# YurongYou/MODEST

Measured on AMD Instinct MI355X. Metric: LiDAR scans/sec through PP-score+cluster seed-label pipeline, higher is better.
Workload: dtype f64

## Files before the change

modest_amd/csrc/cluster.hip:

```cpp
#include "common.h"
#include "compact.h"
#include "mask_pred.h"
#include <cmath>

using namespace modest;

namespace {

constexpr int CG = 128;
constexpr int CG_CELLS = CG * CG;
constexpr int WPB = 4;
constexpr int KNN_KEYS = 1024;
constexpr double D_INF = __builtin_huge_val();

struct CGrid {
    double ox, oy, inv_c;
};

__device__ __forceinline__ int cg_coord(float v, double o, double inv_c) {
    double f = floor(((double)v - o) * inv_c);
    f = fmin(fmax(f, 0.0), (double)(CG - 1));
    return (int)f;
}

__global__ __launch_bounds__(1024) void cg_bbox(const float *__restrict__ xyz, int n, double c, CGrid *g,
                                                unsigned *__restrict__ zeroed, int zero_words) {
    for (int i = threadIdx.x; i < zero_words; i += blockDim.x) zeroed[i] = 0u;
    float mnx = INFINITY, mny = INFINITY, mxx = -INFINITY, mxy = -INFINITY;
    for (int i = threadIdx.x; i < n; i += blockDim.x) {
        const float x = xyz[3 * (size_t)i], y = xyz[3 * (size_t)i + 1];
        mnx = fminf(mnx, x);
        mxx = fmaxf(mxx, x);
        mny = fminf(mny, y);
        mxy = fmaxf(mxy, y);
    }
    for (int o = 32; o > 0; o >>= 1) {
        mnx = fminf(mnx, __shfl_xor(mnx, o));
        mxx = fmaxf(mxx, __shfl_xor(mxx, o));
        mny = fminf(mny, __shfl_xor(mny, o));
        mxy = fmaxf(mxy, __shfl_xor(mxy, o));
    }
    __shared__ float s[4][16];
    const int w = threadIdx.x >> 6, l = threadIdx.x & 63;
    if (l == 0) {
        s[0][w] = mnx;
        s[1][w] = mxx;
        s[2][w] = mny;
        s[3][w] = mxy;
    }
    __syncthreads();
    if (threadIdx.x == 0) {
        for (int k = 1; k < 16; ++k) {
            s[0][0] = fminf(s[0][0], s[0][k]);
            s[1][0] = fmaxf(s[1][0], s[1][k]);
            s[2][0] = fminf(s[2][0], s[2][k]);
            s[3][0] = fmaxf(s[3][0], s[3][k]);
        }
        double cx = 0.5 * ((double)s[0][0] + (double)s[1][0]);
        double cy = 0.5 * ((double)s[2][0] + (double)s[3][0]);
        if (!(cx == cx) || fabs(cx) > 1e30) cx = 0.0;
        if (!(cy == cy) || fabs(cy) > 1e30) cy = 0.0;
        g->ox = cx - 0.5 * CG * c;
        g->oy = cy - 0.5 * CG * c;
        g->inv_c = 1.0 / c;
    }
}

__global__ void cg_count(const float *__restrict__ xyz, int n, const CGrid *g, unsigned *cnt) {
    const int i = blockIdx.x * blockDim.x + threadIdx.x;
    if (i >= n) return;
    const int cx = cg_coord(xyz[3 * (size_t)i], g->ox, g->inv_c);
    const int cy = cg_coord(xyz[3 * (size_t)i + 1], g->oy, g->inv_c);
    atomicAdd(&cnt[cy * CG + cx], 1u);
}

constexpr int SCAN_IPT = 8;
template <bool CELLS>
__device__ __forceinline__ void scan_u32_body(const unsigned *in, unsigned *__restrict__ out, int n,
                                              unsigned *__restrict__ total_copy, const int *__restrict__ flag_src,
                                              unsigned *__restrict__ cursor, unsigned *clear_in, unsigned *flags) {
    __shared__ unsigned tile[16][64 * (SCAN_IPT + 1)];
    __shared__ unsigned wtot[2][16];
    const int lane = threadIdx.x & 63, w = threadIdx.x >> 6;
    unsigned *T = tile[w];
    unsigned carry = 0;
    int buf = 0;
    for (int t0 = 0; t0 < n; t0 += 1024 * SCAN_IPT, buf ^= 1) {
        const int seg = t0 + w * 64 * SCAN_IPT;
        unsigned v[SCAN_IPT];
#pragma unroll
        for (int q = 0; q < SCAN_IPT; ++q) {
            const int e = q * 64 + lane;
            v[q] = seg + e < n ? in[seg + e] : 0u;
        }
#pragma unroll
// ... 49 lines not shown
        out[n] = carry;
        if (total_copy) {
            total_copy[0] = flag_src ? (unsigned)*flag_src : 0u;
            total_copy[1] = carry;
        }
    }
}
template <bool CELLS>
__global__ __launch_bounds__(1024) void scan_u32(const unsigned *in, unsigned *__restrict__ out, int n,
                                                 unsigned *__restrict__ total_copy = nullptr,
                                                 const int *__restrict__ flag_src = nullptr,
                                                 unsigned *__restrict__ cursor = nullptr,
                                                 unsigned *clear_in = nullptr, unsigned *flags = nullptr) {
    scan_u32_body<CELLS>(in, out, n, total_copy, flag_src, cursor, clear_in, flags);
}

__device__ __forceinline__ void cg_scatter_body(const float *__restrict__ xyz, const float *__restrict__ pp, int n, const CGrid *g, unsigned *cursor, float4 *__restrict__ sorted, int *__restrict__ sidx, const int *__restrict__ idx, const float *__restrict__ inten_src, const float *__restrict__ rows, int stride, float *__restrict__ sortedI, const unsigned bx, const unsigned gx) {
    const int i = bx * blockDim.x + threadIdx.x;
    if (i >= n) return;
    const float x = xyz[3 * (size_t)i], y = xyz[3 * (size_t)i + 1], z = xyz[3 * (size_t)i + 2];
    const int cell = cg_coord(y, g->oy, g->inv_c) * CG + cg_coord(x, g->ox, g->inv_c);
    const unsigned slot = atomicAdd(&cursor[cell], 1u);
    const int src = idx ? idx[i] : i;
    sorted[slot] = make_float4(x, y, z, pp[src]);
    sidx[slot] = i;
    if (sortedI) sortedI[slot] = rows ? rows[(size_t)src * stride + 3] : inten_src[src];
}
__global__  void cg_scatter(const float *__restrict__ xyz, const float *__restrict__ pp, int n, const CGrid *g, unsigned *cursor, float4 *__restrict__ sorted, int *__restrict__ sidx, const int *__restrict__ idx, const float *__restrict__ inten_src, const float *__restrict__ rows, int stride, float *__restrict__ sortedI) {
    cg_scatter_body(xyz, pp, n, g, cursor, sorted, sidx, idx, inten_src, rows, stride, sortedI, blockIdx.x, gridDim.x);
}

__device__ __forceinline__ void mask_count_kernel_body(const float *__restrict__ pts, int n, int stride, MaskParams P, CGrid G, CGrid *__restrict__ g, unsigned *cnt, int *__restrict__ labels, float *__restrict__ kept, int *__restrict__ kept_idx, unsigned long long *state, int *n_kept, const unsigned bx, const unsigned gx) {
    const unsigned blk = compact_ticket(state);
    const long long i = (long long)blk * 1024 + threadIdx.x;
    if (blk == 0 && threadIdx.x == 0) *g = G;
    bool keep = false;
    float x = 0, y = 0, z = 0;
    if (i < n) {
        const float *p = pts + i * stride;
        x = p[0];
        y = p[1];
        z = p[2];
        keep = mask_keep(P, x, y, z);
        labels[i] = -1;
        if (keep) atomicAdd(&cnt[cg_coord(y, G.oy, G.inv_c) * CG + cg_coord(x, G.ox, G.inv_c)], 1u);
    }
    const unsigned long long dst = compact_offset(keep, blk, gx, state, n_kept);
    if (keep) {
        kept[3 * dst + 0] = x;
        kept[3 * dst + 1] = y;
        kept[3 * dst + 2] = z;
        kept_idx[dst] = (int)i;
    }
}
__global__ __launch_bounds__(1024) void mask_count_kernel(const float *__restrict__ pts, int n, int stride, MaskParams P, CGrid G, CGrid *__restrict__ g, unsigned *cnt, int *__restrict__ labels, float *__restrict__ kept, int *__restrict__ kept_idx, unsigned long long *state, int *n_kept) {
    mask_count_kernel_body(pts, n, stride, P, G, g, cnt, labels, kept, kept_idx, state, n_kept, blockIdx.x, gridDim.x);
}

__device__ __forceinline__ double dist2(const float4 &a, const float4 &b) {
    const double dx = (double)a.x - (double)b.x;
    const double dy = (double)a.y - (double)b.y;
    const double dz = (double)a.z - (double)b.z;
    return __dadd_rn(__dadd_rn(__dmul_rn(dx, dx), __dmul_rn(dy, dy)), __dmul_rn(dz, dz));
}

struct Rows {
    static constexpr int n = 3;
    unsigned s[3], e[3];
};
__device__ __forceinline__ Rows rows_of(const float4 &q, const CGrid *g, const unsigned *__restrict__ start) {
    const int cx = cg_coord(q.x, g->ox, g->inv_c), cy = cg_coord(q.y, g->oy, g->inv_c);
    const int x0 = max(cx - 1, 0), x1 = min(cx + 1, CG - 1);
    Rows r;
#pragma unroll
    for (int d = 0; d < 3; ++d) {
        const int yy = cy - 1 + d;
        const bool ok = yy >= 0 && yy < CG;
        r.s[d] = ok ? start[yy * CG + x0] : 0u;
        r.e[d] = ok ? start[yy * CG + x1 + 1] : 0u;
    }
    return r;
}

__device__ __forceinline__ void knn_kth_kernel_body(const float4 *__restrict__ sorted, int n, const CGrid *g, const unsigned *__restrict__ start, int k, double r2, double *__restrict__ kthS, const unsigned bx, const unsigned gx) {
    __shared__ unsigned hist_all[WPB][256];
    __shared__ unsigned keys_all[WPB][KNN_KEYS];
    const int w = threadIdx.x >> 6, lane = threadIdx.x & 63;
    const int s = bx * WPB + w;
    if (s >= n) return;
    unsigned *hist = hist_all[w];
    unsigned *keys = keys_all[w];
    const float4 q = sorted[s];
    const Rows R = rows_of(q, g, start);
    unsigned prefix = 0, mask = 0, cntF = 0;
    int kk = k - 1;
    bool enough = true;
    unsigned nkeys = 0;
    for (int shift = 24; shift >= 0; shift -= 8) {
        for (int b = lane; b < 256; b += 64) hist[b] = 0;
        __builtin_amdgcn_wave_barrier();
        if (shift == 24) {
    #pragma unroll
    for (int r = 0; r < R.n; ++r)
            for (unsigned base = R.s[r]; base < R.e[r]; base += 64) {
                const unsigned j = base + lane;
                bool inr = false;
                unsigned key = 0;
                if (j < R.e[r] && (int)j != s) {
                    const double d2 = dist2(q, sorted[j]);
                    inr = d2 <= r2;
                    key = __float_as_uint((float)d2);
                }
                const unsigned long long bal = __ballot(inr);
                if (inr) {
                    atomicAdd(&hist[(key >> 24) & 255u], 1u);
                    const unsigned pos = nkeys + (unsigned)__popcll(bal & ((1ULL << lane) - 1ULL));
                    if (pos < (unsigned)KNN_KEYS) keys[pos] = key;
                }
                nkeys += (unsigned)__popcll(bal);
            }
        } else if (nkeys <= (unsigned)KNN_KEYS) {
            for (unsigned i = lane; i < nkeys; i += 64) {
                const unsigned key = keys[i];
                if ((key & mask) == prefix) atomicAdd(&hist[(key >> shift) & 255u], 1u);
            }
        } else {
    #pragma unroll
    for (int r = 0; r < R.n; ++r)
            for (unsigned j = R.s[r] + lane; j < R.e[r]; j += 64) {
                if ((int)j == s) continue;
                const double d2 = dist2(q, sorted[j]);
                if (d2 <= r2) {
                    const unsigned key = __float_as_uint((float)d2);
                    if ((key & mask) == prefix) atomicAdd(&hist[(key >> shift) & 255u], 1u);
                }
            }
        }
        __builtin_amdgcn_wave_barrier();
        const unsigned c0 = hist[4 * lane], c1 = hist[4 * lane + 1], c2 = hist[4 * lane + 2],
                       c3 = hist[4 * lane + 3];
        const unsigned mine = c0 + c1 + c2 + c3;
        unsigned inc = mine;
        for (int o = 1; o < 64; o <<= 1) {
            const unsigned v = __shfl_up(inc, o);
            if (lane >= o) inc += v;
        }
        const unsigned total = __shfl(inc, 63);
        if (shift == 24 && total < (unsigned)k) {
            enough = false;
            break;
        }
        const unsigned long long bal = __ballot(inc > (unsigned)kk);
        const int owner = __ffsll((long long)bal) - 1;
        const unsigned excl = __shfl(inc - mine, owner);
        const unsigned o0 = __shfl(c0, owner), o1 = __shfl(c1, owner), o2 = __shfl(c2, owner),
                       o3 = __shfl(c3, owner);
        int rem = kk - (int)excl;
        int bin = 4 * owner;
        cntF = o0;
        if (rem >= (int)o0) {
            rem -= o0;
            ++bin;
            cntF = o1;
            if (rem >= (int)o1) {
                rem -= o1;
                ++bin;
                cntF = o2;
                if (rem >= (int)o2) {
                    rem -= o2;
                    ++bin;
                    cntF = o3;
                }
            }
        }
        kk = rem;
        prefix |= (unsigned)bin << shift;
        mask |= 255u << shift;
        __builtin_amdgcn_wave_barrier();
    }
    double result = D_INF;
    if (enough) {
        double lo = -1.0;
        for (;;) {
            double m = D_INF;
        #pragma unroll
    for (int r = 0; r < R.n; ++r)
                for (unsigned j = R.s[r] + lane; j < R.e[r]; j += 64) {
                    if ((int)j == s) continue;
                    const double d2 = dist2(q, sorted[j]);
                    if (d2 <= r2 && d2 > lo && __float_as_uint((float)d2) == prefix) m = fmin(m, d2);
                }
            for (int o = 32; o > 0; o >>= 1) m = fmin(m, __shfl_xor(m, o));
            if (cntF == 1) {
                result = m;
                break;
            }
            unsigned c = 0;
        #pragma unroll
    for (int r = 0; r < R.n; ++r)
                for (unsigned j = R.s[r] + lane; j < R.e[r]; j += 64)
                    if ((int)j != s && dist2(q, sorted[j]) == m) ++c;
            for (int o = 32; o > 0; o >>= 1) c += __shfl_xor(c, o);
            if (kk < (int)c || c == 0) {
                result = m;
                break;
            }
            kk -= (int)c;
            lo = m;
        }
    }
    if (lane == 0) kthS[s] = result;
}
__global__ __launch_bounds__(64 * WPB) void knn_kth_kernel(const float4 *__restrict__ sorted, int n, const CGrid *g, const unsigned *__restrict__ start, int k, double r2, double *__restrict__ kthS) {
    knn_kth_kernel_body(sorted, n, g, start, k, r2, kthS, blockIdx.x, gridDim.x);
}

struct EdgeP {
    double r2, eps;
    int use_knn, affinity;
    const float *inten;
};

__device__ __forceinline__ bool weight_ok(const float4 &q, const float4 &c, const EdgeP &ep, int s, unsigned j) {
    float w;
    if (ep.affinity == 0) {
        w = fabsf(q.w - c.w);
    } else if (ep.affinity == 1) {
        const float d = q.w - c.w;
        w = (float)exp((double)(d * d));
    } else {
        const float dx = q.x - c.x, dy = q.y - c.y, dz = q.z - c.z, di = ep.inten[s] - ep.inten[j];
        w = sqrtf(((dx * dx + dy * dy) + dz * dz) + di * di);
    }
    return (double)w <= ep.eps;
}

__device__ __forceinline__ bool edge_ok(const float4 &q, double kq, const float4 &c, double kc, const EdgeP &ep,
                                        int s, unsigned j) {
    const double d2 = dist2(q, c);
    const double lim = ep.use_knn ? fmin(fmin(kq, kc), ep.r2) : ep.r2;
    if (!(d2 <= lim)) return false;
    return weight_ok(q, c, ep, s, j);
}

__global__ __launch_bounds__(64 * WPB) void degree_kernel(const float4 *__restrict__ sorted, int n,
                                                          const CGrid *g,
                                                          const unsigned *__restrict__ start,
                                                          const double *__restrict__ kthS, EdgeP ep, int min_samples,
                                                          unsigned char *__restrict__ coreS) {
    const int w = threadIdx.x >> 6, lane = threadIdx.x & 63;
    const int s = blockIdx.x * WPB + w;
    if (s >= n) return;
    const float4 q = sorted[s];
    const double kq = kthS[s];
    const Rows R = rows_of(q, g, start);
    unsigned cnt = 0;
#pragma unroll
    for (int r = 0; r < R.n; ++r)
        for (unsigned j = R.s[r] + lane; j < R.e[r]; j += 64) {
            if ((int)j == s) continue;
            if (edge_ok(q, kq, sorted[j], kthS[j], ep, s, j)) ++cnt;
        }
    for (int o = 32; o > 0; o >>= 1) cnt += __shfl_xor(cnt, o);
    if (lane == 0) coreS[s] = ((int)cnt + 1 >= min_samples) ? 1 : 0;
}

__device__ __forceinline__ int uf_load(int *p, int i) {
    return __hip_atomic_load(p + i, __ATOMIC_RELAXED, __HIP_MEMORY_SCOPE_AGENT);
}
__device__ __forceinline__ int uf_find(int *parent, int x) {
    int p = uf_load(parent, x);
    while (p != x) {
        const int gp = uf_load(parent, p);
        if (gp != p) __hip_atomic_store(parent + x, gp, __ATOMIC_RELAXED, __HIP_MEMORY_SCOPE_AGENT);
        x = p;
        p = gp;
    }
    return x;
}
__device__ __forceinline__ void uf_unite(int *parent, int a, int b) {
    for (;;) {
        a = uf_find(parent, a);
        b = uf_find(parent, b);
        if (a == b) return;
        if (a > b) {
            const int t = a;
            a = b;
            b = t;
        }
        const int old = atomicCAS(parent + b, b, a);
        if (old == b) return;
    }
}

__global__ void uf_init(int *parent, int n) {
    const int i = blockIdx.x * blockDim.x + threadIdx.x;
    if (i < n) parent[i] = i;
}

__global__ __launch_bounds__(64 * WPB) void hook_min_kernel(const float4 *__restrict__ sorted, int n,
                                                            const CGrid *g,
                                                            const unsigned *__restrict__ start,
                                                            const double *__restrict__ kthS,
                                                            const unsigned char *__restrict__ coreS,
                                                            const int *__restrict__ sidx, EdgeP ep, int *parent) {
    const int w = threadIdx.x >> 6, lane = threadIdx.x & 63;
    const int s = blockIdx.x * WPB + w;
    if (s >= n) return;
    if (!coreS[s]) return;
    const float4 q = sorted[s];
    const double kq = kthS[s];
    const int me = sidx[s];
    const Rows R = rows_of(q, g, start);
    int best = me;
#pragma unroll
    for (int r = 0; r < R.n; ++r)
        for (unsigned j = R.s[r] + lane; j < R.e[r]; j += 64) {
            if ((int)j == s || !coreS[j]) continue;
            const int other = sidx[j];
            if (other < best && edge_ok(q, kq, sorted[j], kthS[j], ep, s, j)) best = other;
        }
    for (int o = 32; o > 0; o >>= 1) best = min(best, __shfl_xor(best, o));
    if (lane == 0) parent[me] = best;
}

__global__ __launch_bounds__(64 * WPB) void union_kernel(const float4 *__restrict__ sorted, int n,
                                                         const CGrid *g,
                                                         const unsigned *__restrict__ start,
                                                         const double *__restrict__ kthS,
                                                         const unsigned char *__restrict__ coreS,
                                                         const int *__restrict__ sidx, EdgeP ep, int *parent) {
    const int w = threadIdx.x >> 6, lane = threadIdx.x & 63;
    const int s = blockIdx.x * WPB + w;
    if (s >= n) return;
    if (!coreS[s]) return;
    const float4 q = sorted[s];
    const double kq = kthS[s];
    const int me = sidx[s];
    const Rows R = rows_of(q, g, start);
#pragma unroll
    for (int r = 0; r < R.n; ++r)
        for (unsigned j = R.s[r] + lane; j < R.e[r]; j += 64) {
            if ((int)j <= s) continue;
            if (!coreS[j]) continue;
            if (edge_ok(q, kq, sorted[j], kthS[j], ep, s, j)) uf_unite(parent, me, sidx[j]);
        }
}

__global__ void compress_kernel(int *parent, const unsigned char *__restrict__ coreS,
                                const int *__restrict__ sidx, int n, int *__restrict__ root,
                                unsigned *__restrict__ isroot) {
    const int s = blockIdx.x * blockDim.x + threadIdx.x;
    if (s >= n) return;
    const int i = sidx[s];
    const int r = uf_find(parent, i);
    root[i] = r;
    isroot[i] = (coreS[s] && r == i) ? 1u : 0u;
}

__global__ __launch_bounds__(64 * WPB) void label_kernel(const float4 *__restrict__ sorted, int n,
                                                         const CGrid *g,
                                                         const unsigned *__restrict__ start,
                                                         const double *__restrict__ kthS,
                                                         const unsigned char *__restrict__ coreS,
                                                         const int *__restrict__ sidx,
                                                         const int *__restrict__ root,
                                                         const unsigned *__restrict__ rank, EdgeP ep, int *__restrict__ labels,
                                                         const int *__restrict__ oidx) {
    const int w = threadIdx.x >> 6, lane = threadIdx.x & 63;
    const int s = blockIdx.x * WPB + w;
    if (s >= n) return;
    const int me = sidx[s];
    if (coreS[s]) {
        if (lane == 0) labels[oidx ? oidx[me] : me] = (int)rank[root[me]];
        return;
    }
    const float4 q = sorted[s];
    const double kq = kthS[s];
    const Rows R = rows_of(q, g, start);
    int best = 0x7fffffff;
#pragma unroll
    for (int r = 0; r < R.n; ++r)
        for (unsigned j = R.s[r] + lane; j < R.e[r]; j += 64) {
            if ((int)j == s || !coreS[j]) continue;
            if (edge_ok(q, kq, sorted[j], kthS[j], ep, s, j)) best = min(best, root[sidx[j]]);
        }
    for (int o = 32; o > 0; o >>= 1) best = min(best, __shfl_xor(best, o));
    if (lane == 0) labels[oidx ? oidx[me] : me] = (best == 0x7fffffff) ? -1 : (int)rank[best];
}

constexpr int ADJ = 128;
constexpr int AG = 16;

constexpr int UF_NONE = 0x7fffffff;
template <bool ORIG>
__device__ __forceinline__ void degree_adj_kernel_body(const float4 *__restrict__ sorted, int n, const CGrid *g,
                                                       const unsigned *__restrict__ start,
                                                       const double *__restrict__ kthS, const EdgeP &ep, int min_samples,
                                                       unsigned char *__restrict__ coreS, int *__restrict__ deg,
                                                       int *__restrict__ adj, int *overflow,
                                                       const int *__restrict__ sidx, int *__restrict__ parent,
                                                       const unsigned bx) {
    const int w = threadIdx.x >> 6, lane = threadIdx.x & 63;
    const int s = bx * WPB + w;
    if (s >= n) return;
    if (!ORIG && lane == 0) parent[sidx[s]] = sidx[s];
    const float4 q = sorted[s];
    const double kq = kthS[s];
    const Rows R = rows_of(q, g, start);
    unsigned total = 0;
#pragma unroll
    for (int r = 0; r < R.n; ++r)
        for (unsigned base = R.s[r]; base < R.e[r]; base += 128) {
            const unsigned j0 = base + lane, j1 = j0 + 64;
            const bool in0 = j0 < R.e[r], in1 = j1 < R.e[r];
            const unsigned a0 = in0 ? j0 : (unsigned)s, a1 = in1 ? j1 : (unsigned)s;
            const float4 c0 = sorted[a0], c1 = sorted[a1];
            const double k0 = kthS[a0], k1 = kthS[a1];
            const bool e0 = in0 && (int)j0 != s && edge_ok(q, kq, c0, k0, ep, s, j0);
            const bool e1 = in1 && (int)j1 != s && edge_ok(q, kq, c1, k1, ep, s, j1);
            const unsigned long long b0 = __ballot(e0), b1 = __ballot(e1);
            const unsigned p0 = total + __popcll(b0 & ((1ULL << lane) - 1ULL));
            const unsigned p1 = total + __popcll(b0) + __popcll(b1 & ((1ULL << lane) - 1ULL));
            if (e0 && p0 < (unsigned)ADJ) adj[(size_t)s * ADJ + p0] = ORIG ? sidx[j0] : (int)j0;
            if (e1 && p1 < (unsigned)ADJ) adj[(size_t)s * ADJ + p1] = ORIG ? sidx[j1] : (int)j1;
            total += __popcll(b0) + __popcll(b1);
        }
    if (lane == 0) {
        deg[s] = (int)min(total, (unsigned)ADJ);
        coreS[s] = ((int)total + 1 >= min_samples) ? 1 : 0;
        if (ORIG) parent[sidx[s]] = ((int)total + 1 >= min_samples) ? sidx[s] : UF_NONE;
        if (total > (unsigned)ADJ) atomicOr(overflow, 1);
    }
}
template <bool ORIG>
__global__ __launch_bounds__(64 * WPB) void degree_adj_kernel(const float4 *__restrict__ sorted, int n,
                                                              const CGrid *g,
                                                              const unsigned *__restrict__ start,
                                                              const double *__restrict__ kthS, EdgeP ep, int min_samples,
                                                              unsigned char *__restrict__ coreS,
                                                              int *__restrict__ deg, int *__restrict__ adj,
                                                              int *overflow, const int *__restrict__ sidx,
                                                              int *__restrict__ parent) {
    degree_adj_kernel_body<ORIG>(sorted, n, g, start, kthS, ep, min_samples, coreS, deg, adj, overflow, sidx, parent, blockIdx.x);
}

__global__ void hook_adj_kernel(int n, int stride, const unsigned char *__restrict__ coreS, const int *__restrict__ deg,
                                const int *__restrict__ adj, const int *__restrict__ sidx, int *parent) {
    const int t = blockIdx.x * blockDim.x + threadIdx.x;
    const int s = t / AG, sub = t % AG;
    const bool on = s < n && coreS[s];
    int rme = 0, m = 0x7fffffff;
    if (on) {
        rme = parent[sidx[s]];
        m = rme;
        const int *row = adj + (size_t)s * stride;
        const int d = deg[s];
        for (int e = sub; e < d; e += AG) {
            const int j = row[e];
            if (coreS[j]) m = min(m, parent[sidx[j]]);
        }
    }
    for (int o = AG / 2; o > 0; o >>= 1) m = min(m, __shfl_xor(m, o));
    if (on && sub == 0 && m < rme) atomicMin(parent + rme, m);
}

__global__ void flatten_kernel(int *parent, int n) {
    const int i = blockIdx.x * blockDim.x + threadIdx.x;
    if (i >= n) return;
    int r = uf_load(parent, i);
    for (;;) {
        const int p = uf_load(parent, r);
        if (p == r) break;
        r = p;
    }
    __hip_atomic_store(parent + i, r, __ATOMIC_RELAXED, __HIP_MEMORY_SCOPE_AGENT);
}

__global__ void union_adj_kernel(int n, int stride, const unsigned char *__restrict__ coreS, const int *__restrict__ deg,
                                 const int *__restrict__ adj, const int *__restrict__ sidx, int *parent) {
    const int t = blockIdx.x * blockDim.x + threadIdx.x;
    const int s = t / AG, sub = t % AG;
    if (s >= n || !coreS[s]) return;
    const int me = sidx[s];
    const int *row = adj + (size_t)s * stride;
    const int d = deg[s];
    for (int e = sub; e < d; e += AG) {
        const int j = row[e];
        if (j <= s || !coreS[j]) continue;
        const int other = sidx[j];
        if (uf_load(parent, me) != uf_load(parent, other)) uf_unite(parent, me, other);
    }
}

__global__ void label_adj_kernel(int n, int stride, const unsigned char *__restrict__ coreS, const int *__restrict__ deg,
                                 const int *__restrict__ adj, const int *__restrict__ sidx,
                                 const int *__restrict__ root, const unsigned *__restrict__ rank,
                                 int *__restrict__ labels, const int *__restrict__ oidx) {
    const int t = blockIdx.x * blockDim.x + threadIdx.x;
    const int s = t / AG, sub = t % AG;
    const bool on = s < n;
    const bool core = on && coreS[s];
    int best = 0x7fffffff;
    if (on && !core) {
        const int *row = adj + (size_t)s * stride;
        const int d = deg[s];
        for (int e = sub; e < d; e += AG) {
            const int j = row[e];
            if (coreS[j]) best = min(best, root[sidx[j]]);
        }
    }
    for (int o = AG / 2; o > 0; o >>= 1) best = min(best, __shfl_xor(best, o));
    if (!on || sub) return;
    const int me = sidx[s];
    labels[oidx ? oidx[me] : me] = core ? (int)rank[root[me]] : (best == 0x7fffffff) ? -1 : (int)rank[best];
}

__device__ __forceinline__ void hook_orig_kernel_body(int n, const unsigned char *__restrict__ coreS, const int *__restrict__ deg, const int *__restrict__ adj, const int *__restrict__ sidx, int *parent, const unsigned bx, const unsigned gx) {
    const int t = bx * blockDim.x + threadIdx.x;
    const int s = t / AG, sub = t % AG;
    const bool on = s < n && coreS[s];
    int rme = 0, m = UF_NONE;
    if (on) {
        rme = parent[sidx[s]];
        m = rme;
        const int *row = adj + (size_t)s * ADJ;
        const int d = deg[s];
// ... 314 lines not shown
    unsigned char *coreS = A.take<unsigned char>(n);
    int *parent = A.take<int>(n);
    int *root = A.take<int>(n);
    unsigned *isroot = A.take<unsigned>(n);
    unsigned *rank = A.take<unsigned>(n + 1);
    int *deg = A.take<int>(n);
    int *adj = A.take<int>((size_t)n * (unbounded ? (ustride > ADJ ? ustride : ADJ) : ADJ));
    float *sortedI = A.take<float>(n);
    int *degOut = A.take<int>(n);
    int *Lmin = A.take<int>(n);
    int *overflow = reinterpret_cast<int *>(zeroed + CG_CELLS);
    unsigned *h_res = reinterpret_cast<unsigned *>(ctx->pinned);
    const int *oidx = pre ? pre->idx : nullptr;

    const double c = radius * (1.0 + 1.0 / 1024.0);
    const double r2 = radius * radius;
    const int nb = (n + 255) / 256, nw = (n + WPB - 1) / WPB;
    const int nbA = (int)(((long long)n * AG + 255) / 256);
    const bool l2 = affinity_type == MODEST_AFFINITY_L2_4D;
    if (pre) {
        g = pre->g;
        scan_u32<true><<<1, 1024, 0, stream>>>(pre->cnt, start, CG_CELLS, nullptr, nullptr, cursor, pre->cnt,
                                               reinterpret_cast<unsigned *>(overflow));
        cg_scatter<<<nb, 256, 0, stream>>>(xyz, pp, n, g, cursor, sorted, sidx, pre->idx, nullptr, pre->rows, pre->stride,
                                           l2 ? sortedI : nullptr);
    } else {
        cg_bbox<<<1, 1024, 0, stream>>>(xyz, n, c, g, zeroed, (int)zero_words);
        cg_count<<<nb, 256, 0, stream>>>(xyz, n, g, cnt);
        scan_u32<true><<<1, 1024, 0, stream>>>(cnt, start, CG_CELLS, nullptr, nullptr, cursor, nullptr, nullptr);
        cg_scatter<<<nb, 256, 0, stream>>>(xyz, pp, n, g, cursor, sorted, sidx, nullptr, intensity, nullptr, 0,
                                           l2 ? sortedI : nullptr);
    }
    EdgeP ep;
    ep.r2 = r2;
    ep.eps = eps;
    ep.use_knn = neighbor_type == MODEST_GRAPH_RADIUS_MUTUAL_KNN;
    ep.affinity = affinity_type;
    ep.inten = sortedI;
    if (unbounded) {
        int *changed = overflow + 1;
        knn_kth_unbounded_kernel<<<nw, 64 * WPB, 0, stream>>>(sorted, n, g, start, k_neighbors, c, kthS);
        adj_knn_kernel<<<nw, 64 * WPB, 0, stream>>>(sorted, n, g, start, kthS, ep, c,
                                                   neighbor_type == MODEST_GRAPH_MUTUAL_KNN, ustride, degOut, adj,
                                                   overflow);
        MODEST_HIP_CHECK(hipMemcpyAsync(deg, degOut, (size_t)n * 4, hipMemcpyDeviceToDevice, stream));
        if (neighbor_type == MODEST_GRAPH_SYM_KNN)
            adj_symmetrize_kernel<<<nb, 256, 0, stream>>>(sorted, n, kthS, ustride, degOut, deg, adj, overflow);
        core_from_deg_kernel<<<nb, 256, 0, stream>>>(n, deg, ustride, min_samples, coreS, deg);
        if (neighbor_type == MODEST_GRAPH_KNN) {
            dir_init_kernel<<<nb, 256, 0, stream>>>(n, coreS, sidx, Lmin);
            for (int it = 0; it < 4096; ++it) {
                dir_push_kernel<<<nbA, 256, 0, stream>>>(n, ustride, coreS, deg, adj, Lmin, changed);
                if (it % 8 == 7) {
                    MODEST_HIP_CHECK(hipMemcpyAsync(ctx->pinned + 16, changed, 4, hipMemcpyDeviceToHost, stream));
                    MODEST_HIP_CHECK(hipMemsetAsync(changed, 0, 4, stream));
                    MODEST_HIP_CHECK(hipStreamSynchronize(stream));
                    if (!*reinterpret_cast<int *>(ctx->pinned + 16)) break;
                }
            }
            dir_roots_kernel<<<nb, 256, 0, stream>>>(n, coreS, sidx, Lmin, root, isroot);
            scan_u32<false><<<1, 1024, 0, stream>>>(isroot, rank, n, h_res, overflow);
            dir_label_kernel<<<nb, 256, 0, stream>>>(n, root, rank, labels, oidx);
        } else {
            uf_init<<<nb, 256, 0, stream>>>(parent, n);
            for (int round = 0; round < HOOK_ROUNDS; ++round) {
                hook_adj_kernel<<<nbA, 256, 0, stream>>>(n, ustride, coreS, deg, adj, sidx, parent);
                flatten_kernel<<<nb, 256, 0, stream>>>(parent, n);
            }
            union_adj_kernel<<<nbA, 256, 0, stream>>>(n, ustride, coreS, deg, adj, sidx, parent);
            compress_kernel<<<nb, 256, 0, stream>>>(parent, coreS, sidx, n, root, isroot);
            scan_u32<false><<<1, 1024, 0, stream>>>(isroot, rank, n, h_res, overflow);
            label_adj_kernel<<<nbA, 256, 0, stream>>>(n, ustride, coreS, deg, adj, sidx, root, rank, labels, oidx);
        }
        MODEST_HIP_CHECK(hipGetLastError());
        MODEST_HIP_CHECK(hipStreamSynchronize(stream));
        MODEST_REQUIRE(!h_res[0],
                       "k-NN graph: a row exceeded its capacity (massively tied k-th distances or a hub point)");
        if (n_clusters) *n_clusters = (int32_t)h_res[1];
        if (kth_d2) scatter_kth<<<nb, 256, 0, stream>>>(kthS, sidx, n, kth_d2);
        MODEST_HIP_CHECK(hipGetLastError());
        return MODEST_OK;
    }
    if (ep.use_knn || kth_d2)
        knn_kth_kernel<<<nw, 64 * WPB, 0, stream>>>(sorted, n, g, start, k_neighbors, r2, kthS);
    degree_adj_kernel<true><<<nw, 64 * WPB, 0, stream>>>(sorted, n, g, start, kthS, ep, min_samples, coreS, deg, adj,
                                                        overflow, sidx, parent);
    for (int round = 0; round < HOOK_ROUNDS; ++round) {
        hook_orig_kernel<<<nbA, 256, 0, stream>>>(n, coreS, deg, adj, sidx, parent);
        flatten_orig_kernel<<<nb, 256, 0, stream>>>(parent, n);
    }
    union_orig_kernel<<<nbA, 256, 0, stream>>>(n, coreS, deg, adj, sidx, parent);
    compress_orig_kernel<<<nb, 256, 0, stream>>>(parent, coreS, sidx, n, root, isroot);
    scan_u32<false><<<1, 1024, 0, stream>>>(isroot, rank, n, h_res, overflow);
    label_orig_kernel<<<nbA, 256, 0, stream>>>(n, coreS, deg, adj, sidx, root, rank, labels, oidx);
    MODEST_HIP_CHECK(hipGetLastError());
    {
        MODEST_HIP_CHECK(hipStreamSynchronize(stream));
        if (h_res[0]) {
            cluster_overflow_path(sorted, n, g, start, kthS, ep, min_samples, coreS, parent, sidx, root, isroot, rank, h_res,
                                  overflow, labels, oidx, stream);
            MODEST_HIP_CHECK(hipStreamSynchronize(stream));
        }
        if (n_clusters) *n_clusters = (int32_t)h_res[1];
    }
    if (kth_d2) scatter_kth<<<nb, 256, 0, stream>>>(kthS, sidx, n, kth_d2);
    MODEST_HIP_CHECK(hipGetLastError());
    return MODEST_OK;
}

}

extern "C" int modest_cluster_dbscan_ex(modest_ctx *ctx, const float *xyz, const float *pp,
                                        const float *intensity, int n, int neighbor_type, int affinity_type,
                                        int k_neighbors, double radius, double eps, int min_samples,
                                        int32_t *labels, double *kth_d2, int32_t *n_clusters,
                                        void *stream_) {
    MODEST_REQUIRE(ctx != nullptr, "ctx is NULL");
    MODEST_REQUIRE(n >= 0, "n < 0");
    MODEST_REQUIRE(k_neighbors >= 1 && radius > 0.0 && min_samples >= 1, "bad parameters");
    MODEST_REQUIRE(neighbor_type >= MODEST_GRAPH_RADIUS_MUTUAL_KNN && neighbor_type <= MODEST_GRAPH_MUTUAL_KNN,
                   "neighbor_type out of range");
    const bool unbounded = neighbor_type >= MODEST_GRAPH_KNN;
    MODEST_REQUIRE(!unbounded || n == 0 || n > k_neighbors, "k-NN graph: n_neighbors must be < n (sklearn raises too)");
    MODEST_REQUIRE(affinity_type >= MODEST_AFFINITY_L1 && affinity_type <= MODEST_AFFINITY_L2_4D,
                   "affinity_type must be l1, exp or 3d_l2_distance");
    MODEST_REQUIRE(affinity_type != MODEST_AFFINITY_L2_4D || intensity != nullptr || n == 0,
                   "3d_l2_distance needs the intensity column (the reference takes the norm of the (n,4) rows)");
    if (n_clusters) *n_clusters = 0;
    if (n == 0) return MODEST_OK;
    MODEST_REQUIRE(xyz && pp && labels, "NULL buffer");
    hipStream_t stream = as_stream(stream_);
    MODEST_HIP_CHECK(hipSetDevice(ctx->device));
    int rc = modest_ctx_reserve(ctx, cluster_arena_bytes(n, neighbor_type, k_neighbors));
    if (rc) return rc;
    rc = modest_ctx_reserve_pinned(ctx, 64);
    if (rc) return rc;
    return cluster_impl(ctx, 0, xyz, pp, intensity, n, neighbor_type, affinity_type, k_neighbors, radius, eps,
                        min_samples, labels, kth_d2, n_clusters, stream, nullptr);
}

int modest_mask_cluster_phase(modest_ctx *ctx, const float *pts, int n, int stride, const float *pp,
                              const double *plane4, double offset, const double *only_range4,
                              const double *limit_range4, int neighbor_type, int affinity_type, int k_neighbors,
                              double radius, double eps, int min_samples, int32_t *labels, int32_t *n_kept,
                              int32_t *n_clusters, void *stream_, int phase) {
    MODEST_REQUIRE(ctx != nullptr, "ctx is NULL");
    MODEST_REQUIRE(n >= 0 && (stride == 3 || stride == 4), "bad n/stride");
    MODEST_REQUIRE(plane4 && limit_range4 && n_kept, "NULL argument");
    MODEST_REQUIRE(k_neighbors >= 1 && radius > 0.0 && min_samples >= 1, "bad parameters");
    MODEST_REQUIRE(neighbor_type >= MODEST_GRAPH_RADIUS_MUTUAL_KNN && neighbor_type <= MODEST_GRAPH_MUTUAL_KNN,
                   "neighbor_type out of range");
    MODEST_REQUIRE(affinity_type >= MODEST_AFFINITY_L1 && affinity_type <= MODEST_AFFINITY_L2_4D,
                   "affinity_type must be l1, exp or 3d_l2_distance");
    MODEST_REQUIRE(affinity_type != MODEST_AFFINITY_L2_4D || stride == 4,
                   "3d_l2_distance needs the intensity column of the scan rows");
    if (phase & 1) {
        *n_kept = 0;
        if (n_clusters) *n_clusters = 0;
    }
    if (n == 0) return MODEST_OK;
    MODEST_REQUIRE(pts && pp && labels, "NULL buffer");
    hipStream_t stream = as_stream(stream_);
    MODEST_HIP_CHECK(hipSetDevice(ctx->device));
    const size_t own = arena_sz((size_t)n * 12) + arena_sz((size_t)n * 4) + arena_sz(sizeof(CGrid));
    int rc = modest_ctx_reserve(ctx, own + cluster_arena_bytes(n, neighbor_type, k_neighbors));
    if (rc) return rc;
    rc = modest_ctx_reserve_pinned(ctx, 256);
    if (rc) return rc;
    Arena A(ctx->scratch);
// ... 47 lines not shown
    rc = cluster_impl(ctx, own, kept, pp, nullptr, m, neighbor_type, affinity_type, k_neighbors, radius, eps, min_samples,
                      labels, nullptr, n_clusters, stream, &pre);
    if (rc == MODEST_OK) ctx->zwords_dirty = 0;
    return rc;
}

extern "C" int modest_mask_cluster(modest_ctx *ctx, const float *pts, int n, int stride, const float *pp,
                                   const double *plane4, double offset, const double *only_range4,
                                   const double *limit_range4, int neighbor_type, int affinity_type, int k_neighbors,
                                   double radius, double eps, int min_samples, int32_t *labels, int32_t *n_kept,
                                   int32_t *n_clusters, void *stream_) {
    return modest_mask_cluster_phase(ctx, pts, n, stride, pp, plane4, offset, only_range4, limit_range4, neighbor_type,
                                     affinity_type, k_neighbors, radius, eps, min_samples, labels, n_kept, n_clusters,
                                     stream_, 3);
}

extern "C" int modest_cluster_dbscan(modest_ctx *ctx, const float *xyz, const float *pp, int n,
                                     int k_neighbors, double radius, double eps, int min_samples,
                                     int32_t *labels, double *kth_d2, int32_t *n_clusters,
                                     void *stream_) {
    return modest_cluster_dbscan_ex(ctx, xyz, pp, nullptr, n, MODEST_GRAPH_RADIUS_MUTUAL_KNN, MODEST_AFFINITY_L1,
                                    k_neighbors, radius, eps, min_samples, labels, kth_d2, n_clusters, stream_);
}

#include "mask_chain.h"
#include <algorithm>
#include <cstring>
#include <vector>

namespace {
struct MCB {
    const float *pts, *pp;
    MaskParams P;
    CGrid G;
    CGrid *g;
    unsigned *cnt;
    int *labels;
    float *kept;
    int *kept_idx;
    unsigned long long *state;
    int *h_kept;
    unsigned *start, *cursor, *flags;
    float4 *sorted;
    int *sidx;
    double *kthS;
    unsigned char *coreS;
    int *parent, *root;
    unsigned *isroot, *rank;
    int *deg, *adj;
    unsigned *h_res;
    const double *plane_dev;
    int n, stride, nblk, m, nb, nw, nbA, pad;
};

__global__ __launch_bounds__(1024) void mcb_mask_count(const MCB *__restrict__ tab) {
    const MCB &S = tab[blockIdx.y];
    if ((int)blockIdx.x >= S.nblk) return;
    MaskParams P = S.P;
    if (S.plane_dev) {
        P.n0 = S.plane_dev[0];
        P.n1 = S.plane_dev[1];
        P.n2 = S.plane_dev[2];
        P.d = S.plane_dev[3];
        P.norm = sqrt((P.n0 * P.n0 + P.n1 * P.n1) + P.n2 * P.n2);
    }
    mask_count_kernel_body(S.pts, S.n, S.stride, P, S.G, S.g, S.cnt, S.labels, S.kept, S.kept_idx, S.state, S.h_kept,
                           blockIdx.x, (unsigned)S.nblk);
}
template <bool CELLS>
__global__ __launch_bounds__(1024) void mcb_scan(const MCB *__restrict__ tab) {
    const MCB &S = tab[blockIdx.y];
    if (S.m <= 0) return;
    if (CELLS)
        scan_u32_body<true>(S.cnt, S.start, CG_CELLS, nullptr, nullptr, S.cursor, S.cnt, S.flags);
    else
        scan_u32_body<false>(S.isroot, S.rank, S.m, S.h_res, reinterpret_cast<const int *>(S.flags), nullptr, nullptr, nullptr);
}
__global__ void mcb_cg_scatter(const MCB *__restrict__ tab) {
    const MCB &S = tab[blockIdx.y];
    if ((int)blockIdx.x >= S.nb) return;
    cg_scatter_body(S.kept, S.pp, S.m, S.g, S.cursor, S.sorted, S.sidx, S.kept_idx, nullptr, S.pts, S.stride, nullptr,
                    blockIdx.x, (unsigned)S.nb);
}
__global__ __launch_bounds__(64 * WPB) void mcb_knn_kth(const MCB *__restrict__ tab, int k, double r2) {
    const MCB &S = tab[blockIdx.y];
    if ((int)blockIdx.x >= S.nw) return;
    knn_kth_kernel_body(S.sorted, S.m, S.g, S.start, k, r2, S.kthS, blockIdx.x, (unsigned)S.nw);
}
__global__ __launch_bounds__(64 * WPB) void mcb_degree_adj(const MCB *__restrict__ tab, EdgeP ep, int min_samples) {
    const MCB &S = tab[blockIdx.y];
    if ((int)blockIdx.x >= S.nw) return;
    degree_adj_kernel_body<true>(S.sorted, S.m, S.g, S.start, S.kthS, ep, min_samples, S.coreS, S.deg, S.adj,
                                 reinterpret_cast<int *>(S.flags), S.sidx, S.parent, blockIdx.x);
}
__global__ void mcb_hook(const MCB *__restrict__ tab) {
    const MCB &S = tab[blockIdx.y];
    if ((int)blockIdx.x >= S.nbA) return;
    hook_orig_kernel_body(S.m, S.coreS, S.deg, S.adj, S.sidx, S.parent, blockIdx.x, (unsigned)S.nbA);
}
__global__ void mcb_flatten(const MCB *__restrict__ tab) {
    const MCB &S = tab[blockIdx.y];
    if ((int)blockIdx.x >= S.nb) return;
    flatten_orig_kernel_body(S.parent, S.m, blockIdx.x, (unsigned)S.nb);
}
__global__ void mcb_union(const MCB *__restrict__ tab) {
    const MCB &S = tab[blockIdx.y];
    if ((int)blockIdx.x >= S.nbA) return;
    union_orig_kernel_body(S.m, S.coreS, S.deg, S.adj, S.sidx, S.parent, blockIdx.x, (unsigned)S.nbA);
}
__global__ void mcb_compress(const MCB *__restrict__ tab) {
    const MCB &S = tab[blockIdx.y];
    if ((int)blockIdx.x >= S.nb) return;
    compress_orig_kernel_body(S.parent, S.coreS, S.sidx, S.m, S.root, S.isroot, blockIdx.x, (unsigned)S.nb);
}
__global__ void mcb_label(const MCB *__restrict__ tab) {
    const MCB &S = tab[blockIdx.y];
    if ((int)blockIdx.x >= S.nbA) return;
    label_orig_kernel_body(S.m, S.coreS, S.deg, S.adj, S.sidx, S.root, S.rank, S.labels, S.kept_idx, blockIdx.x,
                           (unsigned)S.nbA);
}

int mcb_upload(modest_ctx *ctx0, const std::vector<MCB> &tab, hipStream_t stream, const MCB **dev) {
    char *d = nullptr, *h = nullptr;
    const size_t bytes = tab.size() * sizeof(MCB);
    int rc = modest_ctx_chain_tab(ctx0, bytes, &d);
    if (rc) return rc;
    rc = modest_ctx_stage_slot(ctx0, bytes, reinterpret_cast<void **>(&h));
    if (rc) return rc;
    memcpy(h, tab.data(), bytes);
    MODEST_HIP_CHECK(hipMemcpyAsync(d, h, bytes, hipMemcpyHostToDevice, stream));
    rc = modest_ctx_stage_commit(ctx0, stream);
    if (rc) return rc;
    *dev = reinterpret_cast<const MCB *>(d);
    return MODEST_OK;
}
}

bool modest_mask_chain_supported(int neighbor_type, int affinity_type) {
    return (neighbor_type == MODEST_GRAPH_RADIUS_MUTUAL_KNN || neighbor_type == MODEST_GRAPH_RADIUS) &&
           affinity_type != MODEST_AFFINITY_L2_4D;
}

struct modest_mask_chain_state {
    std::vector<MCB> tab;
    std::vector<size_t> own;
};

int modest_mask_chain_count(modest_mask_chain_scan *S, int B, double offset, const double *only_range4,
                            const double *limit_range4, int neighbor_type, int k_neighbors, double radius,
                            modest_mask_chain_state **state_out, hipStream_t stream) {
    MODEST_REQUIRE(S != nullptr && B >= 1 && B <= 64 && limit_range4 != nullptr && state_out != nullptr, "bad chain");
    auto *st = new modest_mask_chain_state;
    *state_out = st;
    st->tab.resize((size_t)B);
    st->own.resize((size_t)B);
    const double c = radius * (1.0 + 1.0 / 1024.0);
    int maxblk = 1;
    for (int s = 0; s < B; ++s) {
        modest_mask_chain_scan &q = S[s];
        MCB &b = st->tab[(size_t)s];
        memset(&b, 0, sizeof(b));
        q.n_kept = q.n_clusters = 0;
        q.alone = 0;
        MODEST_REQUIRE(q.ctx && q.pts && q.pp && q.labels && (q.plane4 || q.plane4_dev) && q.n >= 1 && (q.stride == 3 || q.stride == 4),
                       "bad scan of the chain");
        modest_ctx *ctx = q.ctx;
        const size_t own = arena_sz((size_t)q.n * 12) + arena_sz((size_t)q.n * 4) + arena_sz(sizeof(CGrid));
        st->own[(size_t)s] = own;
        int rc = modest_ctx_reserve(ctx, own + cluster_arena_bytes(q.n, neighbor_type, k_neighbors));
        if (rc) return rc;
        rc = modest_ctx_reserve_pinned(ctx, 256);
        if (rc) return rc;
        Arena A(ctx->scratch);
        b.kept = A.take<float>((size_t)q.n * 3);
        b.kept_idx = A.take<int>(q.n);
        b.g = A.take<CGrid>(1);
// ... 18 lines not shown
        if (rc) return rc;
        b.pts = q.pts;
        b.pp = q.pp;
        b.labels = q.labels;
        b.n = q.n;
        b.stride = q.stride;
        maxblk = std::max(maxblk, b.nblk);
    }
    const MCB *dev = nullptr;
    int rc = mcb_upload(S[0].ctx, st->tab, stream, &dev);
    if (rc) return rc;
    mcb_mask_count<<<dim3((unsigned)maxblk, (unsigned)B), 1024, 0, stream>>>(dev);
    MODEST_HIP_CHECK(hipGetLastError());
    return MODEST_OK;
}

void modest_mask_chain_free(modest_mask_chain_state *st) { delete st; }

int modest_mask_chain_cluster(modest_mask_chain_scan *S, int B, modest_mask_chain_state *st, int neighbor_type,
                              int affinity_type, int k_neighbors, double radius, double eps, int min_samples,
                              hipStream_t stream) {
    MODEST_REQUIRE(S != nullptr && st != nullptr && (int)st->tab.size() == B, "bad chain");
    const double r2 = radius * radius;
    EdgeP ep;
    ep.r2 = r2;
    ep.eps = eps;
    ep.use_knn = neighbor_type == MODEST_GRAPH_RADIUS_MUTUAL_KNN;
    ep.affinity = affinity_type;
    ep.inten = nullptr;
    int maxnb = 1, maxnw = 1, maxnbA = 1, live = 0;
    for (int s = 0; s < B; ++s) {
        modest_mask_chain_scan &q = S[s];
        MCB &b = st->tab[(size_t)s];
        modest_ctx *ctx = q.ctx;
        ctx->zwords_live = 0;
        const int m = *b.h_kept;
        q.n_kept = m;
        b.m = m;
        if (q.alone) {
            b.m = 0;
            continue;
        }
        if (m == 0) {
            ctx->zwords_dirty = 0;
            continue;
        }
        if (neighbor_type != MODEST_GRAPH_RADIUS && m <= k_neighbors) {
            q.alone = 1;
            b.m = 0;
            continue;
        }
        ++live;
        Arena A(ctx->scratch + st->own[(size_t)s]);
        A.take<CGrid>(1);
        unsigned *zeroed = A.take<unsigned>((size_t)CG_CELLS + 4);
        b.start = A.take<unsigned>(CG_CELLS + 1);
        b.cursor = A.take<unsigned>(CG_CELLS + 1);
        b.sorted = A.take<float4>(m);
        b.sidx = A.take<int>(m);
        b.kthS = A.take<double>(m);
        b.coreS = A.take<unsigned char>(m);
        b.parent = A.take<int>(m);
        b.root = A.take<int>(m);
        b.isroot = A.take<unsigned>(m);
        b.rank = A.take<unsigned>(m + 1);
        b.deg = A.take<int>(m);
        b.adj = A.take<int>((size_t)m * ADJ);
        b.flags = zeroed + CG_CELLS;
        b.h_res = reinterpret_cast<unsigned *>(ctx->pinned);
        b.nb = (m + 255) / 256;
        b.nw = (m + WPB - 1) / WPB;
        b.nbA = (int)(((long long)m * AG + 255) / 256);
        maxnb = std::max(maxnb, b.nb);
        maxnw = std::max(maxnw, b.nw);
        maxnbA = std::max(maxnbA, b.nbA);
    }
    if (live == 0) return MODEST_OK;
    const MCB *dev = nullptr;
    int rc = mcb_upload(S[0].ctx, st->tab, stream, &dev);
    if (rc) return rc;
    const unsigned Bu = (unsigned)B;
    mcb_scan<true><<<dim3(1, Bu), 1024, 0, stream>>>(dev);
    mcb_cg_scatter<<<dim3((unsigned)maxnb, Bu), 256, 0, stream>>>(dev);
    if (ep.use_knn) mcb_knn_kth<<<dim3((unsigned)maxnw, Bu), 64 * WPB, 0, stream>>>(dev, k_neighbors, r2);
    mcb_degree_adj<<<dim3((unsigned)maxnw, Bu), 64 * WPB, 0, stream>>>(dev, ep, min_samples);
    for (int round = 0; round < HOOK_ROUNDS; ++round) {
        mcb_hook<<<dim3((unsigned)maxnbA, Bu), 256, 0, stream>>>(dev);
        mcb_flatten<<<dim3((unsigned)maxnb, Bu), 256, 0, stream>>>(dev);
    }
    mcb_union<<<dim3((unsigned)maxnbA, Bu), 256, 0, stream>>>(dev);
    mcb_compress<<<dim3((unsigned)maxnb, Bu), 256, 0, stream>>>(dev);
    mcb_scan<false><<<dim3(1, Bu), 1024, 0, stream>>>(dev);
    mcb_label<<<dim3((unsigned)maxnbA, Bu), 256, 0, stream>>>(dev);
    MODEST_HIP_CHECK(hipGetLastError());
    MODEST_HIP_CHECK(hipStreamSynchronize(stream));
    bool again = false;
    for (int s = 0; s < B; ++s) {
        MCB &b = st->tab[(size_t)s];
        if (b.m == 0) continue;
        if (b.h_res[0]) {
            cluster_overflow_path(b.sorted, b.m, b.g, b.start, b.kthS, ep, min_samples, b.coreS, b.parent, b.sidx, b.root,
                                  b.isroot, b.rank, b.h_res, reinterpret_cast<int *>(b.flags), b.labels, b.kept_idx, stream);
            again = true;
        }
    }
    if (again) MODEST_HIP_CHECK(hipStreamSynchronize(stream));
    for (int s = 0; s < B; ++s) {
        MCB &b = st->tab[(size_t)s];
        if (b.m == 0) continue;
        S[s].n_clusters = (int32_t)b.h_res[1];
        S[s].ctx->zwords_dirty = 0;
    }
    return MODEST_OK;
}

extern "C" void modest_warm_cluster(void) {
    hipFuncAttributes a;
    (void)hipFuncGetAttributes(&a, reinterpret_cast<const void *>(cg_count));
}
```

Baseline: 7749.

## Emit candidate neighbor lists during kNN pass and filter them for degree

The kNN k-th-distance kernel now records, on its first sweep over the 3x3 grid cells, every neighbor within radius whose distance key is at or below the final radix prefix and that passes the weight test, into the adjacency row. A new degree_from_knn kernel then filters only those stored candidates with the full edge test instead of rescanning the grid neighborhood. The goal is to avoid a second spatial neighbor scan with its distance recomputation when use_knn is set. In exchange the kNN kernel does extra ballot/stores, and rows capped at ADJ entries can set the overflow flag and force the slow fallback path.

```diff
diff --git a/modest_amd/csrc/cluster.hip b/modest_amd/csrc/cluster.hip
--- a/modest_amd/csrc/cluster.hip
+++ b/modest_amd/csrc/cluster.hip
@@ -11,6 +11,7 @@
 constexpr int CG_CELLS = CG * CG;
 constexpr int WPB = 4;
 constexpr int KNN_KEYS = 1024;
+constexpr int ADJ = 128;
 constexpr double D_INF = __builtin_huge_val();
 
 struct CGrid {
@@ -226,7 +227,27 @@
     return r;
 }
 
-__device__ __forceinline__ void knn_kth_kernel_body(const float4 *__restrict__ sorted, int n, const CGrid *g, const unsigned *__restrict__ start, int k, double r2, double *__restrict__ kthS, const unsigned bx, const unsigned gx) {
+struct EdgeP {
+    double r2, eps;
+    int use_knn, affinity;
+    const float *inten;
+};
+
+__device__ __forceinline__ bool weight_ok(const float4 &q, const float4 &c, const EdgeP &ep, int s, unsigned j) {
+    float w;
+    if (ep.affinity == 0) {
+        w = fabsf(q.w - c.w);
+    } else if (ep.affinity == 1) {
+        const float d = q.w - c.w;
+        w = (float)exp((double)(d * d));
+    } else {
+        const float dx = q.x - c.x, dy = q.y - c.y, dz = q.z - c.z, di = ep.inten[s] - ep.inten[j];
+        w = sqrtf(((dx * dx + dy * dy) + dz * dz) + di * di);
+    }
+    return (double)w <= ep.eps;
+}
+
+__device__ __forceinline__ void knn_kth_kernel_body(const float4 *__restrict__ sorted, int n, const CGrid *g, const unsigned *__restrict__ start, int k, double r2, double *__restrict__ kthS, const EdgeP &ep, int *__restrict__ deg, int *__restrict__ adj, int *overflow, const unsigned bx, const unsigned gx) {
     __shared__ unsigned hist_all[WPB][256];
     __shared__ unsigned keys_all[WPB][KNN_KEYS];
     const int w = threadIdx.x >> 6, lane = threadIdx.x & 63;
@@ -323,17 +344,37 @@
         __builtin_amdgcn_wave_barrier();
     }
     double result = D_INF;
-    if (enough) {
+    const bool emit = ep.use_knn != 0;
+    unsigned nrow = 0;
+    if (!enough) prefix = 0xffffffffu;
+    if (enough || emit) {
         double lo = -1.0;
+        bool first = emit;
         for (;;) {
             double m = D_INF;
         #pragma unroll
     for (int r = 0; r < R.n; ++r)
-                for (unsigned j = R.s[r] + lane; j < R.e[r]; j += 64) {
-                    if ((int)j == s) continue;
-                    const double d2 = dist2(q, sorted[j]);
-                    if (d2 <= r2 && d2 > lo && __float_as_uint((float)d2) == prefix) m = fmin(m, d2);
+                for (unsigned base = R.s[r]; base < R.e[r]; base += 64) {
+                    const unsigned j = base + lane;
+                    bool cand = false;
+                    if (j < R.e[r] && (int)j != s) {
+                        const float4 c = sorted[j];
+                        const double d2 = dist2(q, c);
+                        if (d2 <= r2) {
+                            const unsigned key = __float_as_uint((float)d2);
+                            if (d2 > lo && key == prefix) m = fmin(m, d2);
+                            cand = first && key <= prefix && (ep.affinity == 1 || weight_ok(q, c, ep, s, j));
+                        }
+                    }
+                    if (first) {
+                        const unsigned long long bal = __ballot(cand);
+                        const unsigned pos = nrow + (unsigned)__popcll(bal & ((1ULL << lane) - 1ULL));
+                        if (cand && pos < (unsigned)ADJ) adj[(size_t)s * ADJ + pos] = (int)j;
+                        nrow += (unsigned)__popcll(bal);
+                    }
                 }
+            first = false;
+            if (!enough) break;
             for (int o = 32; o > 0; o >>= 1) m = fmin(m, __shfl_xor(m, o));
             if (cntF == 1) {
                 result = m;
@@ -353,30 +394,16 @@
             lo = m;
         }
     }
-    if (lane == 0) kthS[s] = result;
-}
-__global__ __launch_bounds__(64 * WPB) void knn_kth_kernel(const float4 *__restrict__ sorted, int n, const CGrid *g, const unsigned *__restrict__ start, int k, double r2, double *__restrict__ kthS) {
-    knn_kth_kernel_body(sorted, n, g, start, k, r2, kthS, blockIdx.x, gridDim.x);
-}
-
-struct EdgeP {
-    double r2, eps;
-    int use_knn, affinity;
-    const float *inten;
-};
-
-__device__ __forceinline__ bool weight_ok(const float4 &q, const float4 &c, const EdgeP &ep, int s, unsigned j) {
-    float w;
-    if (ep.affinity == 0) {
-        w = fabsf(q.w - c.w);
-    } else if (ep.affinity == 1) {
-        const float d = q.w - c.w;
-        w = (float)exp((double)(d * d));
-    } else {
-        const float dx = q.x - c.x, dy = q.y - c.y, dz = q.z - c.z, di = ep.inten[s] - ep.inten[j];
-        w = sqrtf(((dx * dx + dy * dy) + dz * dz) + di * di);
-    }
-    return (double)w <= ep.eps;
+    if (lane == 0) {
+        kthS[s] = result;
+        if (emit) {
+            deg[s] = (int)min(nrow, (unsigned)ADJ);
+            if (nrow > (unsigned)ADJ) atomicOr(overflow, 1);
+        }
+    }
+}
+__global__ __launch_bounds__(64 * WPB) void knn_kth_kernel(const float4 *__restrict__ sorted, int n, const CGrid *g, const unsigned *__restrict__ start, int k, double r2, double *__restrict__ kthS, EdgeP ep, int *__restrict__ deg, int *__restrict__ adj, int *overflow) {
+    knn_kth_kernel_body(sorted, n, g, start, k, r2, kthS, ep, deg, adj, overflow, blockIdx.x, gridDim.x);
 }
 
 __device__ __forceinline__ bool edge_ok(const float4 &q, double kq, const float4 &c, double kc, const EdgeP &ep,
@@ -533,7 +560,6 @@
     if (lane == 0) labels[oidx ? oidx[me] : me] = (best == 0x7fffffff) ? -1 : (int)rank[best];
 }
 
-constexpr int ADJ = 128;
 constexpr int AG = 16;
 
 constexpr int UF_NONE = 0x7fffffff;
@@ -587,6 +613,64 @@
                                                               int *overflow, const int *__restrict__ sidx,
                                                               int *__restrict__ parent) {
     degree_adj_kernel_body<ORIG>(sorted, n, g, start, kthS, ep, min_samples, coreS, deg, adj, overflow, sidx, parent, blockIdx.x);
+}
+
+#ifndef KROW_LANES
+#define KROW_LANES 64
+#endif
+constexpr int KL = KROW_LANES;
+constexpr int KPB = WPB * (64 / KL);
+static_assert(KL == 64 || KL == 32 || KL == 16, "a wavefront holds a whole number of points");
+template <bool ORIG>
+__device__ __forceinline__ void degree_from_knn_body(const float4 *__restrict__ sorted, int n,
+                                                     const double *__restrict__ kthS, const EdgeP &ep, int min_samples,
+                                                     unsigned char *__restrict__ coreS, int *__restrict__ deg,
+                                                     int *adj, const int *__restrict__ sidx, int *__restrict__ parent,
+                                                     const unsigned bx) {
+    constexpr int E = ADJ / KL;
+    const int lane = threadIdx.x & 63, sub = lane % KL, shift = lane - sub;
+    const int s = (int)(bx * KPB) + (int)(threadIdx.x / KL);
+    if (s - shift / KL >= n) return;
+    const bool live = s < n;
+    const int sc = live ? s : 0;
+    if (!ORIG && live && sub == 0) parent[sidx[sc]] = sidx[sc];
+    const float4 q = sorted[sc];
+    const double kq = kthS[sc];
+    const int nc = live ? deg[sc] : 0;
+    int *row = adj + (size_t)sc * ADJ;
+    unsigned j[E];
+    float4 c[E];
+    double kc[E];
+#pragma unroll
+    for (int i = 0; i < E; ++i) j[i] = (i * KL + sub < nc) ? (unsigned)row[i * KL + sub] : (unsigned)sc;
+#pragma unroll
+    for (int i = 0; i < E; ++i) {
+        c[i] = sorted[j[i]];
+        kc[i] = kthS[j[i]];
+    }
+    const unsigned long long below = (1ULL << sub) - 1ULL, all = KL == 64 ? ~0ULL : (1ULL << (KL & 63)) - 1ULL;
+    unsigned total = 0;
+#pragma unroll
+    for (int i = 0; i < E; ++i) {
+        const bool e = i * KL + sub < nc && edge_ok(q, kq, c[i], kc[i], ep, sc, j[i]);
+        const unsigned long long b = (__ballot(e) >> shift) & all;
+        const unsigned p = total + (unsigned)__popcll(b & below);
+        if (e) row[p] = ORIG ? sidx[j[i]] : (int)j[i];
+        total += (unsigned)__popcll(b);
+    }
+    if (live && sub == 0) {
+        deg[s] = (int)total;
+        coreS[s] = ((int)total + 1 >= min_samples) ? 1 : 0;
+        if (ORIG) parent[sidx[s]] = ((int)total + 1 >= min_samples) ? sidx[s] : UF_NONE;
+    }
+}
+template <bool ORIG>
+__global__ __launch_bounds__(64 * WPB) void degree_from_knn_kernel(const float4 *__restrict__ sorted, int n,
+                                                                   const double *__restrict__ kthS, EdgeP ep, int min_samples,
+                                                                   unsigned char *__restrict__ coreS, int *__restrict__ deg,
+                                                                   int *adj, const int *__restrict__ sidx,
+                                                                   int *__restrict__ parent) {
+    degree_from_knn_body<ORIG>(sorted, n, kthS, ep, min_samples, coreS, deg, adj, sidx, parent, blockIdx.x);
 }
 
 __global__ void hook_adj_kernel(int n, int stride, const unsigned char *__restrict__ coreS, const int *__restrict__ deg,
@@ -1067,9 +1151,13 @@
         return MODEST_OK;
     }
     if (ep.use_knn || kth_d2)
-        knn_kth_kernel<<<nw, 64 * WPB, 0, stream>>>(sorted, n, g, start, k_neighbors, r2, kthS);
-    degree_adj_kernel<true><<<nw, 64 * WPB, 0, stream>>>(sorted, n, g, start, kthS, ep, min_samples, coreS, deg, adj,
-                                                        overflow, sidx, parent);
+        knn_kth_kernel<<<nw, 64 * WPB, 0, stream>>>(sorted, n, g, start, k_neighbors, r2, kthS, ep, deg, adj, overflow);
+    if (ep.use_knn)
+        degree_from_knn_kernel<true><<<(n + KPB - 1) / KPB, 64 * WPB, 0, stream>>>(sorted, n, kthS, ep, min_samples, coreS, deg,
+                                                                                  adj, sidx, parent);
+    else
+        degree_adj_kernel<true><<<nw, 64 * WPB, 0, stream>>>(sorted, n, g, start, kthS, ep, min_samples, coreS, deg, adj,
+                                                            overflow, sidx, parent);
     for (int round = 0; round < HOOK_ROUNDS; ++round) {
         hook_orig_kernel<<<nbA, 256, 0, stream>>>(n, coreS, deg, adj, sidx, parent);
         flatten_orig_kernel<<<nb, 256, 0, stream>>>(parent, n);
@@ -1283,16 +1371,22 @@
     cg_scatter_body(S.kept, S.pp, S.m, S.g, S.cursor, S.sorted, S.sidx, S.kept_idx, nullptr, S.pts, S.stride, nullptr,
                     blockIdx.x, (unsigned)S.nb);
 }
-__global__ __launch_bounds__(64 * WPB) void mcb_knn_kth(const MCB *__restrict__ tab, int k, double r2) {
+__global__ __launch_bounds__(64 * WPB) void mcb_knn_kth(const MCB *__restrict__ tab, int k, double r2, EdgeP ep) {
     const MCB &S = tab[blockIdx.y];
     if ((int)blockIdx.x >= S.nw) return;
-    knn_kth_kernel_body(S.sorted, S.m, S.g, S.start, k, r2, S.kthS, blockIdx.x, (unsigned)S.nw);
+    knn_kth_kernel_body(S.sorted, S.m, S.g, S.start, k, r2, S.kthS, ep, S.deg, S.adj, reinterpret_cast<int *>(S.flags),
+                        blockIdx.x, (unsigned)S.nw);
 }
 __global__ __launch_bounds__(64 * WPB) void mcb_degree_adj(const MCB *__restrict__ tab, EdgeP ep, int min_samples) {
     const MCB &S = tab[blockIdx.y];
     if ((int)blockIdx.x >= S.nw) return;
     degree_adj_kernel_body<true>(S.sorted, S.m, S.g, S.start, S.kthS, ep, min_samples, S.coreS, S.deg, S.adj,
                                  reinterpret_cast<int *>(S.flags), S.sidx, S.parent, blockIdx.x);
+}
+__global__ __launch_bounds__(64 * WPB) void mcb_degree_from_knn(const MCB *__restrict__ tab, EdgeP ep, int min_samples) {
+    const MCB &S = tab[blockIdx.y];
+    if ((int)(blockIdx.x * KPB) >= S.m) return;
+    degree_from_knn_body<true>(S.sorted, S.m, S.kthS, ep, min_samples, S.coreS, S.deg, S.adj, S.sidx, S.parent, blockIdx.x);
 }
 __global__ void mcb_hook(const MCB *__restrict__ tab) {
     const MCB &S = tab[blockIdx.y];
@@ -1477,8 +1571,12 @@
     const unsigned Bu = (unsigned)B;
     mcb_scan<true><<<dim3(1, Bu), 1024, 0, stream>>>(dev);
     mcb_cg_scatter<<<dim3((unsigned)maxnb, Bu), 256, 0, stream>>>(dev);
-    if (ep.use_knn) mcb_knn_kth<<<dim3((unsigned)maxnw, Bu), 64 * WPB, 0, stream>>>(dev, k_neighbors, r2);
-    mcb_degree_adj<<<dim3((unsigned)maxnw, Bu), 64 * WPB, 0, stream>>>(dev, ep, min_samples);
+    if (ep.use_knn) {
+        mcb_knn_kth<<<dim3((unsigned)maxnw, Bu), 64 * WPB, 0, stream>>>(dev, k_neighbors, r2, ep);
+        mcb_degree_from_knn<<<dim3((unsigned)((maxnw * WPB + KPB - 1) / KPB), Bu), 64 * WPB, 0, stream>>>(dev, ep, min_samples);
+    } else {
+        mcb_degree_adj<<<dim3((unsigned)maxnw, Bu), 64 * WPB, 0, stream>>>(dev, ep, min_samples);
+    }
     for (int round = 0; round < HOOK_ROUNDS; ++round) {
         mcb_hook<<<dim3((unsigned)maxnbA, Bu), 256, 0, stream>>>(dev);
         mcb_flatten<<<dim3((unsigned)maxnb, Bu), 256, 0, stream>>>(dev);
```

Result: slower. 7355 (-5.1%).
